# fraunhoferhhi/vvdec

Measured on AMD Instinct MI355X. Metric: decoded frames/sec (4K 10-bit RA) on MI355X, synthetic pre-parsed stream, bit-exact vs ref, higher is better.
Workload: dtype int16

## Files before the change

### vvdec_amd/csrc/vvr_api.cpp

```cpp
#include "vvr_host.h"
#include <algorithm>
#include <condition_variable>
#include <cstdio>
#include <cstring>
#include <deque>
#include <map>
#include <memory>
#include <mutex>
#include <thread>
#include <sched.h>
#include <pthread.h>

int vvr_upload_tables();

static std::vector<int> gpuNodeCpus( int device )
{
  std::vector<int> cpus;
  if( const char* e = getenv( "VVR_NO_PIN" ) ) if( atoi( e ) ) return cpus;
  char bus[64] = { 0 };
  if( hipDeviceGetPCIBusId( bus, sizeof( bus ), device ) != hipSuccess ) return cpus;
  for( char* q = bus; *q; q++ ) *q = (char) tolower( *q );
  char path[256]; snprintf( path, sizeof( path ), "/sys/bus/pci/devices/%s/numa_node", bus );
  int node = -1;
  if( FILE* f = fopen( path, "r" ) ) { if( fscanf( f, "%d", &node ) != 1 ) node = -1; fclose( f ); }
// ... 64 lines not shown
  int state = J_QUEUED;
  int rc = VVR_OK; std::string err;
  vvr_picture pic;
  vvr_prepared* q = nullptr;
  RingEntry* ring = nullptr;
  int lane = -1;
  hipEvent_t done = nullptr;
  hipEvent_t doneHost = nullptr;
  bool completed = false, waited = false;
  std::vector<PendingTiming> timings;
  int* errWord = nullptr;
  std::vector<int32_t> dmvr;
  std::vector<vvr_motion> col;
  bool handled = false;
#ifdef VVR_WATCHDOG
  double tSubmit = 0, tPrep = 0, tBuilt = 0, tRing = 0, tReady = 0, tCommit0 = 0, tCommit1 = 0; hipEvent_t tlA = nullptr, tlB = nullptr; int tlPoc = 0, tlType = 0; unsigned long long tlSeq = 0;
#endif
};

struct vvr_context {
  vvr_config cfg;
  int        device = 0;
  std::string err;
  std::vector<hipStream_t> streams;
  hipStream_t copyStream = nullptr;
  std::vector<DevPlanes>   slots;
  std::vector<std::pair<uint16_t, uint16_t>> slotDim;
  std::vector<DevPlanes>   scratchB;
  std::vector<DevPlanes>   scratchR;
  void*      planeMem = nullptr; bool planeMemOwned = false;
  void*      scratchMem = nullptr;
// ... 83 lines not shown

static hipEvent_t takeEvent( vvr_context* c )
{
  if( !c->eventPool.empty() ) { hipEvent_t e = c->eventPool.back(); c->eventPool.pop_back(); return e; }
  hipEvent_t e = nullptr;
  if( hipEventCreateWithFlags( &e, hipEventDisableTiming ) != hipSuccess ) return nullptr;
  return e;
}

static void completeLocked( vvr_context* c, Job& j )
{
  if( j.completed ) return;
#ifdef VVR_WATCHDOG
  if( j.tlA && j.tlB && c->tlBase )
  {
    float a = 0, b = 0; hipEventElapsedTime( &a, c->tlBase, j.tlA ); hipEventElapsedTime( &b, c->tlBase, j.tlB );
    fprintf( stderr, "[vvr timeline] device seq %3llu poc %4d type %d lane %d: %6.2f .. %6.2f  (base event recorded at host %6.2f)\n", j.tlSeq, j.tlPoc, j.tlType, j.lane, a, b, c->tlBaseHost - c->tl0 );
  }
  if( j.tlA ) { hipEventDestroy( j.tlA ); j.tlA = nullptr; } if( j.tlB ) { hipEventDestroy( j.tlB ); j.tlB = nullptr; }
#endif
  for( auto& t : j.timings )
  {
    float ms = 0; hipEventElapsedTime( &ms, t.a, t.b );
    c->stats[t.kernel].launches++; c->stats[t.kernel].ms += ms; c->stats[t.kernel].bytes += t.bytes;
    hipEventDestroy( t.a ); hipEventDestroy( t.b );
  }
  j.timings.clear();
  if( j.errWord && *j.errWord )
  {
    *j.errWord = 0;
    if( j.state == J_COMMITTED ) { j.state = J_FAILED; j.rc = VVR_ERR_DEVICE; j.err = "intra stage: a block waited for its neighbours beyond the bound (dependency that never completed)"; }
  }
  if( j.q && j.q->numDmvr && j.state == J_COMMITTED )
  {
    const int32_t* src = j.ring ? j.ring->dmvrHost : j.q->dmvrHost;
    j.dmvr.assign( src, src + 2 * (size_t) j.q->numDmvr );
  }
  if( j.q && j.q->colHost && j.state == J_COMMITTED ) j.col.assign( j.q->colHost, j.q->colHost + j.q->numCol );
  if( j.ring && j.ring->owner == &j ) { j.ring->owner = nullptr; j.ring->turn += c->ring.size(); }
  if( j.done ) { c->eventPool.push_back( j.done ); j.done = nullptr; }
  if( j.doneHost ) { c->eventPool.push_back( j.doneHost ); j.doneHost = nullptr; }
  j.q = nullptr;
  j.completed = true;
  WD_PROGRESS();
  c->cv.notify_all();
}

struct CommitPlan { int lane; std::vector<hipEvent_t> waits; RefSet refs; std::vector<int> waitInfo; std::vector<hipEvent_t> outExt ; };

static void pruneExternalEventsLocked( vvr_context* c, int slot )
{
  auto& v = c->slotExt[slot];
  v.erase( std::remove_if( v.begin(), v.end(), []( hipEvent_t ev ) { return hipEventQuery( ev ) == hipSuccess; } ), v.end() );
}

static void planCommitLocked( vvr_context* c, Job& job, CommitPlan& plan )
{
  const vvr_pic_header& h = job.q->hdr;
  int lane = -1;
  if( c->prioLane >= 0 && h.slice_type == 2 )
  {
    auto it = c->jobs.find( c->prioJob );
    bool idle = it == c->jobs.end() || it->second->completed;
// ... 4 lines not shown
  plan.lane = lane; plan.waits.clear(); plan.waitInfo.clear();
  job.lane = lane;
  auto waitFor = [&]( int id ) { auto it = c->jobs.find( id ); if( it != c->jobs.end() ) { Job& j = *it->second; if( !j.completed && j.state == J_COMMITTED && j.lane != lane ) { plan.waits.push_back( j.done ); plan.waitInfo.push_back( j.q ? ( j.id * 16 + j.q->hdr.slice_type * 4 ) : -1 ); plan.waitInfo.push_back( j.lane ); } } };
  for( int id : c->slotUsers[h.out_slot] ) waitFor( id );
  plan.outExt.clear();
  for( hipEvent_t ev : c->slotExt[h.out_slot] ) { plan.waits.push_back( ev ); plan.waitInfo.push_back( -2 ); plan.waitInfo.push_back( -1 ); plan.outExt.push_back( ev ); }
  memset( &plan.refs, 0, sizeof( plan.refs ) );
  if( h.slice_type != 2 )
    for( int l = 0; l < 2; l++ ) for( int i = 0; i < h.num_ref[l]; i++ )
    {
      const int slot = h.ref_slot[l][i];
      if( !c->slotUsers[slot].empty() ) waitFor( c->slotUsers[slot][0] );
      for( hipEvent_t ev : c->slotExt[slot] ) if( std::find( plan.waits.begin(), plan.waits.end(), ev ) == plan.waits.end() ) { plan.waits.push_back( ev ); plan.waitInfo.push_back( -2 ); plan.waitInfo.push_back( -1 ); }
      for( int k = 0; k < 3; k++ ) plan.refs.p[l * VVR_MAX_REFS + i][k] = c->slots[slot].p[k];
    }
  job.done = takeEvent( c ); job.doneHost = takeEvent( c );
}

static int enqueuePicture( vvr_context* c, Job& job, const CommitPlan& plan, std::string& err )
{
#undef HIPCHK
#define HIPCHK( ctx, call ) do { hipError_t e_ = ( call ); if( e_ != hipSuccess ) { err = std::string( #call ) + ": " + hipGetErrorString( e_ ); hipStreamSynchronize( ( ctx )->copyStream ); hipStreamSynchronize( ( ctx )->streams[plan.lane] ); return VVR_ERR_DEVICE; } } while( 0 )
  vvr_prepared* q = job.q;
  const vvr_pic_header& h = q->hdr;
  const int lane = plan.lane;
  hipStream_t s = c->streams[lane];
  if( !job.done || !job.doneHost ) { err = "hipEventCreate failed"; return VVR_ERR_DEVICE; }
#ifdef VVR_WATCHDOG
  const double wdA = wdNow();
#endif
  if( job.ring )
  {
    RingEntry& e = *job.ring;
    HIPCHK( c, hipMemcpyAsync( e.dev + e.stagedBegin, e.host + e.stagedBegin, e.stagedEnd - e.stagedBegin, hipMemcpyHostToDevice, c->copyStream ) );
    for( auto& d : e.direct ) HIPCHK( c, hipMemcpyAsync( e.dev + d.off, d.src, d.n, hipMemcpyHostToDevice, c->copyStream ) );
    HIPCHK( c, hipEventRecord( e.copied, c->copyStream ) );
    HIPCHK( c, hipStreamWaitEvent( s, e.copied, 0 ) );
  }
#ifdef VVR_WATCHDOG
  const double wdB = wdNow(); g_wdPart[0] += wdB - wdA; g_wdPartMax[0] = std::max( g_wdPartMax[0], wdB - wdA );
#endif
#ifdef VVR_WATCHDOG
  for( size_t wi = 0; wi < plan.waits.size(); wi++ )
  {
    const double w0 = wdNow(); HIPCHK( c, hipStreamWaitEvent( s, plan.waits[wi], 0 ) ); const double w = wdNow() - w0;
    if( w > 0.5 ) fprintf( stderr, "[vvr] slow wait: picture %d (type %d, lane %d) wait %zu of %zu on job %d (type %d, lane %d): %.2f ms\n", job.id, (int) h.slice_type, lane, wi, plan.waits.size(), plan.waitInfo[2 * wi] >> 4, ( plan.waitInfo[2 * wi] >> 2 ) & 3, plan.waitInfo[2 * wi + 1], w );
  }
#else
  for( hipEvent_t ev : plan.waits ) HIPCHK( c, hipStreamWaitEvent( s, ev, 0 ) );
#endif
#ifdef VVR_WATCHDOG
  const double wdC = wdNow(); g_wdPart[1] += wdC - wdB; g_wdPartMax[1] = std::max( g_wdPartMax[1], wdC - wdB );
  static const bool tlOn = getenv( "VVR_TIMELINE" ) != nullptr;
  if( tlOn && job.ring )
  {
    if( job.tSubmit - c->tl0 > 50 )
    {
      static hipStream_t tlStream = nullptr; if( !tlStream ) hipStreamCreate( &tlStream );
      c->tl0 = job.tSubmit; hipEventCreate( &c->tlBase ); hipEventRecord( c->tlBase, tlStream ); c->tlBaseHost = wdNow();
      fprintf( stderr, "[vvr timeline] ---- (host: ms since the first submit of the burst; device: ms since the base event)\n" );
    }
    hipEventCreate( &job.tlA ); hipEventCreate( &job.tlB ); job.tlPoc = h.poc; job.tlType = h.slice_type; job.tlSeq = job.seq;
    hipEventRecord( job.tlA, s );
  }
#endif
  job.errWord = c->errHost + ( (unsigned) job.id % VVR_ERR_WORDS ); *job.errWord = 0;
  const RefSet& refs = plan.refs;
  DevPlanes A = c->slots[h.out_slot], B = c->scratchB[lane], R = c->scratchR[lane];
  for( int k = 0; k < 3; k++ ) { const int w = k ? h.width >> 1 : h.width, hh = k ? h.height >> 1 : h.height; A.w[k] = B.w[k] = R.w[k] = w; A.h[k] = B.h[k] = R.h[k] = hh; }
  const int stopAfter = c->cfg.stop_after;
  const bool sao = ( h.tool_flags & ( VVR_TOOL_SAO_LUMA | VVR_TOOL_SAO_CHROMA ) ) != 0 && stopAfter != 1 && stopAfter != 2;
  const bool alf = ( h.tool_flags & VVR_TOOL_ALF ) != 0 && stopAfter == 0;
  const bool fused = ( sao || alf ) && sao_alf_fused( q->pic );
  const bool dbOn = !( h.tool_flags & VVR_TOOL_DEBLOCK_OFF ) && stopAfter != 1;
  const bool hop = fused && dbOn;
  const DevPlanes P = ( fused && !hop ) ? B : A;
  auto timedOn = [&]( int k, hipStream_t st, double algoBytes, auto&& fn )
  {
#ifdef VVR_WATCHDOG
    static const int skipMask = getenv( "VVR_SKIP_KERNELS" ) ? atoi( getenv( "VVR_SKIP_KERNELS" ) ) : 0;
    if( skipMask & ( 1 << k ) ) return;
    const double w0 = wdNow();
#endif
    if( c->statsOn ) { PendingTiming t; hipEventCreate( &t.a ); hipEventCreate( &t.b ); t.kernel = k; t.bytes = algoBytes; hipEventRecord( t.a, st ); fn(); hipEventRecord( t.b, st ); job.timings.push_back( t ); }
    else fn();
#ifdef VVR_WATCHDOG
    const double w = wdNow() - w0; g_wdCall[k][0] += w; g_wdCall[k][1] = std::max( g_wdCall[k][1], w ); g_wdCall[k][2] += 1;
#endif
  };
  auto timed = [&]( int k, auto&& fn ) { timedOn( k, s, q->bytes[k], fn ); };
  {
    PrepWork w;
    if( q->numMcCus ) { w.mcCus = q->mcCus; w.numMcCus = q->numMcCus; w.plain = q->mcDev; w.bdof = q->bdofItems; w.dmvr = q->dmvrItems; }
    if( q->lfpOnDevice && dbOn ) { w.lfMaps = true; w.numCu = q->numCu; w.numTu = q->numTu; w.cell = q->lfCell; w.cellC = q->lfCellC; w.mv = q->lfMv; w.ref = q->lfRef; w.sb = q->lfSb; w.numSb = q->numLfSb; }
    if( q->intraLeaf && q->numIntra ) { w.items = q->intraItems; w.numItems = q->numIntra; w.resi = q->resiItems; w.numResi = q->numResi; w.maps = c->leafMaps[lane]; w.mapInts = c->leafMapInts; w.mapW4 = c->leafW4; w.mapH4 = c->leafH4; }
    launch_prep( s, q->pic, w );
  }
  if( q->lfpOnDevice && dbOn ) timed( K_LF_INIT, [&]{ launch_lf_init( s, q->pic, q->numCu, q->numTu, q->lfCell, q->lfCellC, q->lfMv, q->lfRef, q->lfSb, q->numLfSb, q->lfpDev[0], q->lfpDev[1] ); } );
  if( q->numMc + q->numMcDev ) timedOn( K_MC, s, q->bytes[K_MC] - q->bytesBdof, [&]{ launch_mc( s, q->pic, refs, P, q->mcItems, q->numMc, q->mcDev, q->numMcDev, 0 ); } );
  if( q->numBdofItems ) timedOn( K_MC, s, q->bytesBdof, [&]{ launch_mc( s, q->pic, refs, P, nullptr, 0, q->bdofItems, q->numBdofItems, 1 ); } );
  if( q->numDmvrItems )
  {
    int32_t* out = job.ring ? job.ring->dmvrHost : q->dmvrHost;
    memset( out, 0, sizeof( int32_t ) * 2 * (size_t) q->numDmvr );
    timed( K_MC_DMVR, [&]{ launch_mc_dmvr( s, q->pic, refs, P, q->dmvrItems, q->numDmvrItems, out ); } );
  }
  if( q->numAffItems ) timed( K_MC_AFFINE, [&]{ launch_mc_affine( s, q->pic, refs, P, q->affItems, q->numAffItems ); } );
  if( q->numRprItems ) launch_mc_rpr( s, q->pic, refs, P, q->rprItems, q->numRprItems );
  const bool lmcsOn = ( h.tool_flags & VVR_TOOL_LMCS ) != 0;
  for( int k = 0; k < 3; k++ ) if( q->numTb[k] ) timedOn( K_ITRANS, s, q->bytesTb[k], [&]{ launch_itrans( s, q->pic, P, R, q->tbItems[k], q->numTb[k], 16 << k ); } );
  {
    const size_t need = q->intraLeaf ? 0 : intra_sync_ints( q->numActive, q->numIntra );
    if( need > c->syncCap[lane] )
// ... 313 lines not shown
    for( size_t i = 0; i < c->ring.size(); i++ ) fprintf( stderr, "  ring %zu owner %d\n", i, c->ring[i].owner ? c->ring[i].owner->id : -1 );
    for( size_t i = 0; i < c->streams.size(); i++ ) fprintf( stderr, "  stream %zu query %d\n", i, (int) hipStreamQuery( c->streams[i] ) );
    fprintf( stderr, "  copyStream query %d\n", (int) hipStreamQuery( c->copyStream ) );
    fflush( stderr );
    abort();
  }
}
#endif

struct WorkerHelpers : HostHelpers
{
  vvr_context* c; PrepScratch*& spare;
  bool announced = false;
  WorkerHelpers( vvr_context* c_, PrepScratch*& spare_ ) : c( c_ ), spare( spare_ ) {}
  int width() const override { return c->cfg.host_threads; }
  void notInParts() override { if( announced ) { std::lock_guard<std::mutex> lk( c->mu ); c->partsComing--; announced = false; c->cv.notify_all(); } }
  void run( int n, PrepScratch& own, const std::function<void( int, PrepScratch& )>& fn ) override
  {
    struct State { std::mutex mu; std::condition_variable cv; int remaining; } st; st.remaining = n - 1;
    {
      std::lock_guard<std::mutex> lk( c->mu );
      const bool first = announced;
      for( int part = first ? n - 1 : 1; first ? part >= 1 : part < n; part += first ? -1 : 1 )
      {
        auto task = [&st, &fn, part]( PrepScratch& R ) { fn( part, R ); std::lock_guard<std::mutex> l2( st.mu ); st.remaining--; st.cv.notify_all(); };
        if( first ) c->subtasks.push_front( task ); else c->subtasks.push_back( task );
      }
      if( announced ) { c->partsComing--; announced = false; }
      c->cv.notify_all();
    }
    fn( 0, own );
    for( ;; )
    {
      std::function<void( PrepScratch& )> task;
      { std::lock_guard<std::mutex> lk( c->mu ); if( !c->subtasks.empty() ) { task = std::move( c->subtasks.front() ); c->subtasks.pop_front(); } }
      if( !task ) break;
      if( !spare ) { spare = vvr_scratch_create(); vvr_scratch_intra_leaf( spare, c->intraLeaf, c->leafByLevel ); vvr_scratch_warm( spare, c->cfg ); }
      task( *spare );
    }
    std::unique_lock<std::mutex> lk( st.mu );
    st.cv.wait( lk, [&]{ return st.remaining == 0; } );
  }
};
// ... 662 lines not shown
```

### vvdec_amd/csrc/vvr_host.h

```cpp
#pragma once
#include "vvr_device.h"
#include <mutex>
#include <string>
#include <vector>

static inline size_t alignUp( size_t v, size_t a ) { return ( v + a - 1 ) / a * a; }

enum { K_MC, K_MC_DMVR, K_MC_AFFINE, K_LMCS, K_ITRANS, K_INTRA, K_RESI_ADD, K_DEBLOCK_V, K_DEBLOCK_H, K_SAO, K_ALF, K_COPY, K_OUTPUT, K_LF_INIT, K_INTRA_LEAF,
       K_DEBLOCK4, K_ALF_PLANES ,
       K_OUTPUT_FRAME , K_NUM };

struct vvr_prepared {
  vvr_pic_header hdr;
  PicDev   pic;
  McItem*  mcItems = nullptr; int numMc = 0;
  McItem*  mcDev = nullptr; int numMcDev = 0;
  McCuRef* mcCus = nullptr; int numMcCus = 0;
  McItem*  bdofItems = nullptr; int numBdofItems = 0;
  McItem*  dmvrItems = nullptr; int numDmvrItems = 0;
  McItem*  affItems = nullptr; int numAffItems = 0;
  McItem*  rprItems = nullptr; int numRprItems = 0;
  uint32_t numDmvr = 0;
  TbItem*  tbItems[3] = { nullptr, nullptr, nullptr }; int numTb[3] = { 0, 0, 0 };
  IntraItem* intraItems = nullptr; IntraUnit* units = nullptr; int numActive = 0, numIntra = 0;
// ... 32 lines not shown
int          vvr_host_band_pictures();
void         vvr_scratch_intra_leaf( PrepScratch*, bool on, bool byLevel = false );
void         vvr_scratch_parts_for_all( PrepScratch*, bool on );
void         vvr_scratch_destroy( PrepScratch* );
void         vvr_scratch_warm( PrepScratch*, const vvr_config& cfg );

int    vvr_host_validate( const vvr_config& cfg, const vvr_picture* p, std::string& err );
int    vvr_host_validate_header( const vvr_config& cfg, const vvr_picture* p, std::string& err );
int    vvr_host_validate_records( const vvr_config& cfg, const vvr_picture* p, std::string& err );
#include <functional>
struct HostHelpers
{
  virtual ~HostHelpers() {}
  virtual int  width() const = 0;
  virtual void run( int n, PrepScratch& own, const std::function<void( int, PrepScratch& )>& fn ) = 0;
  virtual void notInParts() {}
};
int    vvr_host_build( const vvr_picture* p, PrepScratch& S, size_t* totalBytes, std::string& err, PinnedRanges* pinned = nullptr, HostHelpers* helpers = nullptr, bool validateRecords = false );
void   vvr_host_pack( const PrepScratch& S, char* host );
size_t vvr_host_staged_bytes( const PrepScratch& S );
size_t vvr_host_num_col( const vvr_picture* p );
void   vvr_host_gather_col( const vvr_picture* p, vvr_motion* dst );
void   vvr_host_upload_plan( const PrepScratch& S, std::vector<DirectCopy>& direct, size_t* stagedBegin, size_t* stagedEnd );
void   vvr_host_bind( const PrepScratch& S, vvr_prepared& q, char* devBase );
```

### vvdec_amd/csrc/vvr_prepare.cpp

```cpp
#include "vvr_host.h"
#include "vvr_lf_init.h"
#include <algorithm>
#include <atomic>
#include <chrono>
#include <cstdio>
#include <cstring>
#include <mutex>
#include <condition_variable>

static inline int ilog2i( int v ) { int l = 0; while( ( 1 << l ) < v ) l++; return l; }

struct BBox { int y0 = 255, y1 = 0, c0 = 255, c1 = 0; };
struct ItemH { uint32_t ctu; BBox bb; uint32_t p0, pn; };
struct DepList
{
  enum { INLINE = 8 };
  uint32_t n = 0, cap = INLINE; uint32_t in[INLINE]; uint32_t* heap = nullptr;
  DepList() {}
  DepList( const DepList& o ) { *this = o; }
  DepList( DepList&& o ) noexcept { n = o.n; cap = o.cap; heap = o.heap; memcpy( in, o.in, sizeof( in ) ); o.heap = nullptr; o.n = 0; o.cap = INLINE; }
  DepList& operator=( const DepList& o ) { if( this != &o ) { n = 0; for( uint32_t v : o ) push_back( v ); } return *this; }
  DepList& operator=( DepList&& o ) noexcept { if( this != &o ) { delete[] heap; n = o.n; cap = o.cap; heap = o.heap; memcpy( in, o.in, sizeof( in ) ); o.heap = nullptr; o.n = 0; o.cap = INLINE; } return *this; }
  ~DepList() { delete[] heap; }
  uint32_t* data() { return heap ? heap : in; } const uint32_t* data() const { return heap ? heap : in; }
  uint32_t* begin() { return data(); } uint32_t* end() { return data() + n; } const uint32_t* begin() const { return data(); } const uint32_t* end() const { return data() + n; }
  size_t size() const { return n; } bool empty() const { return n == 0; }
  uint32_t& operator[]( size_t i ) { return data()[i]; } const uint32_t& operator[]( size_t i ) const { return data()[i]; }
  void push_back( uint32_t v ) { if( n == cap ) { uint32_t* h = new uint32_t[2 * cap]; memcpy( h, data(), sizeof( uint32_t ) * n ); delete[] heap; heap = h; cap *= 2; } data()[n++] = v; }
  void resize( size_t k ) { n = (uint32_t) std::min<size_t>( k, n ); }
  void assign( const uint32_t* a, const uint32_t* b ) { n = 0; for( ; a != b; a++ ) push_back( *a ); }
  void clear() { n = 0; }
};
struct UnitH { uint32_t comp, ctu, i0, i1, iA = 0; bool hasCs = false; BBox bb; DepList deps; bool waited = false; int rank = 0; };

struct Part { const void* src; size_t n, off; bool direct; };

struct PrepScratch
{
  const vvr_picture* p = nullptr;
  vvr_pic_header h;
  int ncomp = 0, w4 = 0, h4 = 0, ctu = 0, ctusX = 0, ctusY = 0, numCtu = 0, vpduLog2 = 0, vpdusX = 0, vpdusY = 0;
  bool wpOn = false, cscale = false, lmcs = false;
  std::vector<McItem> mcRpr;
  std::vector<McItem> mc, mcBdof, mcDmvr, mcAff;
  std::vector<McCuRef> mcCus;
  uint32_t devTiles[3] = { 0, 0, 0 };
  std::vector<uint16_t> ctuSubpicV;
  std::vector<vvr_motion> affMv;
  bool lfpOnDevice = false;
  std::vector<LfSbCell> lfSb;
// ... 7 lines not shown
  std::vector<uint32_t> ctuStartV;
  double bytes[K_NUM] = { 0 };
  double bytesBdof = 0, bytesIntraLuma = 0, bytesTb[3] = { 0, 0, 0 };
  std::vector<int32_t> order;
  std::vector<uint8_t> fastCtu;
  std::vector<uint32_t> itemAtE[3];
  uint16_t fastCell[3][32 * 32]; uint32_t fastFirst[3] = { 0, 0, 0 };
  uint32_t epoch = 0;
  size_t cellIdx( int cx, int cy ) const { const int l = h.log2_ctu - 2, m = ( 1 << l ) - 1; return ( ( (size_t) ( cy >> l ) * ctusX + ( cx >> l ) ) << ( 2 * l ) ) | (size_t) ( ( cy & m ) << l ) | (size_t) ( cx & m ); }
  int32_t itemAtGet( int k, size_t cell ) const { const uint32_t v = itemAtE[k][cell]; return ( v >> 22 ) == epoch ? (int32_t) ( v & 0x3fffffu ) : -1; }
  std::vector<UnitH> units, unitsTmp;
  std::vector<uint32_t> csVpduV;
  std::vector<std::pair<uint32_t, uint32_t>> csProdRange;
  std::vector<uint32_t> csProdPool;
  std::vector<IntraUnit> unitsDev;
  int intraWorkgroups = 0, intraWorkgroupsChroma = 0, numLumaUnits = 0;
  std::vector<IntraItem> resiAdd;
  size_t intraChunk = (size_t) 1 << 30;
  std::vector<uint32_t> parent, newIdx, firstOf, perm, inv, unitCount, unitOfItem[3];
  std::vector<uint64_t> sortKey;
  std::vector<int32_t> unitOfRoot, target;
  std::vector<std::vector<uint32_t>> members, groups;
  std::vector<Part> parts;
  size_t total = 0, numDirect = 0;
  int iLfSb, iLfTu, iLfTuC, iLfMotion;
  int iCu, iTu, iCoef, iAffMv, iL0, iL1, iSao, iAlf, iAlfP, iSlices, iLmcs, iSl, iCtuSlice, iCtuTile, iSubpics, iCtuSubpic, iWp, iCsVpdu, iMc, iMcB, iMcD, iMcA, iTb[3], iIntra, iResi, iUnits, iMcCus, iMcDev[3], iRpr, iMcR;
  size_t stagedEndOff = 0;

  void begin( const vvr_picture* pic )
  {
// ... 6 lines not shown
    {
      uint32_t any = 0;
      for( uint32_t i = 0; i < p->num_slices; i++ ) any |= p->slices[i].tool_flags & VVR_SLICE_TOOL_MASK;
      h.tool_flags = ( h.tool_flags & ~(uint32_t) VVR_SLICE_TOOL_MASK ) | any;
    }
    wpOn = ( h.tool_flags & VVR_TOOL_WP ) && h.slice_type != 2;
    w4 = ( h.width + 3 ) >> 2; h4 = ( h.height + 3 ) >> 2; ctu = 1 << h.log2_ctu;
    ctusX = ( h.width + ctu - 1 ) / ctu; ctusY = ( h.height + ctu - 1 ) / ctu; numCtu = ctusX * ctusY;
    lmcs = ( h.tool_flags & VVR_TOOL_LMCS ) != 0;
    cscale = lmcs && ( h.tool_flags & VVR_TOOL_LMCS_CSCALE ) && ncomp == 3;
    vpduLog2 = std::min<int>( 6, h.log2_ctu ); vpdusX = ( h.width + ( 1 << vpduLog2 ) - 1 ) >> vpduLog2; vpdusY = ( h.height + ( 1 << vpduLog2 ) - 1 ) >> vpduLog2;
    mc.clear(); mcBdof.clear(); mcDmvr.clear(); mcAff.clear(); mcRpr.clear(); affMv.clear(); numDmvr = 0;
    lfSb.clear(); lfpOnDevice = ( h.tool_flags & VVR_TOOL_LFP_ON_DEVICE ) && !( h.tool_flags & VVR_TOOL_DEBLOCK_OFF );
    mcCus.clear(); devTiles[0] = devTiles[1] = devTiles[2] = 0;
    for( int k = 0; k < 3; k++ ) { tb[k].clear(); intra[k].clear(); itemH[k].clear(); prodPool[k].clear(); }
    resiAdd.clear(); intraAll.clear(); units.clear(); unitsDev.clear(); csVpduV.clear(); intraFine = false;
    ctuStartV.assign( 3 * (size_t) ( numCtu + 1 ), 0 );
    for( double& b : bytes ) b = 0;
    bytesBdof = bytesIntraLuma = 0; bytesTb[0] = bytesTb[1] = bytesTb[2] = 0;
  }

  size_t orderIdx( int chn, int lx, int ly ) const { const int m = ( 1 << ( h.log2_ctu - 2 ) ) - 1; return ( ( (size_t) chn << ( h.log2_ctu - 2 ) | (size_t) ( ( ly >> 2 ) & m ) ) << ( h.log2_ctu - 2 ) ) | (size_t) ( ( lx >> 2 ) & m ); }
  int unitAvail( int chn, int x, int y, int32_t cur ) const
  {
    const int cs = chn ? 1 : 0, lx = x << cs, ly = y << cs;
    if( x < 0 || y < 0 || lx >= h.width || ly >= h.height ) return 0;
    const uint32_t c = (uint32_t) ( ( ly >> h.log2_ctu ) * ctusX + ( lx >> h.log2_ctu ) );
    if( c != curCtuIdx ) return c < curCtuIdx && sameSliceAndTile( c, curCtuIdx );
    return order[orderIdx( chn, lx, ly )] < cur;
  }

// ... 43 lines not shown
  inline void levLook( int k, int cx0, int cy0, int cx1, int cy1, uint32_t& d ) const
  {
    cx0 = std::max( cx0, 0 ); cy0 = std::max( cy0, 0 ); cx1 = std::min( cx1, w4 - 1 ); cy1 = std::min( cy1, h4 - 1 );
    const uint16_t* m = &levMap[(size_t) k * w4 * h4];
    for( int y = cy0; y <= cy1; y++ ) for( int x = cx0; x <= cx1; x++ ) d = std::max<uint32_t>( d, m[(size_t) y * w4 + x] );
  }
  inline void levOwn( int k, int cx0, int cy0, int cx1, int cy1, uint16_t v )
  {
    cx1 = std::min( cx1, w4 - 1 ); cy1 = std::min( cy1, h4 - 1 );
    uint16_t* m = &levMap[(size_t) k * w4 * h4];
    for( int y = cy0; y <= cy1; y++ ) std::fill( m + (size_t) y * w4 + cx0, m + (size_t) y * w4 + cx1 + 1, v );
  }
  int emitLeafItems( std::string& err );
  int buildWorkLists( std::string& err, uint32_t cu0 = 0, uint32_t cu1 = 0xffffffffu );
  int buildInParts( const vvr_config& cfg, HostHelpers& helpers, bool validate, std::string& err );
  int formUnits();
  int groupUnits();
  int emitUnitTable( std::string& err );
  void layout( PinnedRanges* pinned );
  void foldLongDepLists();
  void rankUnits();
};

PrepScratch* vvr_scratch_create() { return new PrepScratch(); }
void vvr_scratch_parts_for_all( PrepScratch* S, bool on ) { S->partsForAll = on; }
void vvr_scratch_intra_leaf( PrepScratch* S, bool on, bool byLevel ) { S->leafOn = on; S->leafSortOn = byLevel; }
static bool tusAreTheSplitAt32( const vvr_picture* p, const vvr_cu& cu )
{
  const int tw = cu.w < 32 ? cu.w : 32, th = cu.h < 32 ? cu.h : 32, nx = cu.w / tw, ny = cu.h / th;
  if( (int) cu.num_tu != nx * ny || cu.num_tu < 2 ) return false;
// ... 1144 lines not shown
  {
    UnitH& U = merged[newIndexOfGroup[m]];
    for( uint32_t u : groups[m] ) for( uint32_t d : units[u].deps )
    {
      const uint32_t nd = newIndexOfGroup[target[d]];
      if( nd != newIndexOfGroup[m] && std::find( U.deps.begin(), U.deps.end(), nd ) == U.deps.end() ) U.deps.push_back( nd );
    }
  }
  for( int k = 0; k < ncomp; k++ ) intra[k].swap( intraTmp[k] );
  units.swap( merged );
  foldLongDepLists();
  rankUnits();
  return VVR_OK;
}

int PrepScratch::emitUnitTable( std::string& err )
{
  auto bandsLog2 = [&]( const IntraItem& src, int k )
  {
    const int samples = 1 << ( src.lw + src.lh );
    const bool split = samples > IT_SPLIT_SAMPLES && src.mode <= 66 && ( k || ( !( src.flags & IT_F_MIP ) && ( src.flags & IT_F_ISP ) != IT_F_ISP ) );
    int lp = 0;
    if( split ) while( lp < IT_MAX_LPARTS && ( samples >> lp ) > IT_SPLIT_SAMPLES ) lp++;
    return lp;
  };
  {
    uint32_t at = (uint32_t) intraAll.size();
    for( int k = 0; k < 3; k++ )
    {
      const size_t n = intra[k].size();
      itemMap[k].resize( n + 1 );
      uint32_t* im = itemMap[k].data(); const IntraItem* src = intra[k].data();
      for( size_t bi = 0; bi < n; bi++ ) { im[bi] = at; at += 1u << bandsLog2( src[bi], k ); }
      im[n] = at;
    }
    intraAll.resize( at );
  }
  for( int k = 0; k < 3; k++ )
  {
    const size_t n = intra[k].size();
    const uint32_t* im = itemMap[k].data(); const IntraItem* srcs = intra[k].data(); IntraItem* out = intraAll.data();
    for( size_t bi = 0; bi < n; bi++ )
    {
      const IntraItem& src = srcs[bi];
      const uint32_t indepBlocks = std::min<uint32_t>( src.comp >> 2, (uint32_t) bi );
      const uint32_t indepItems = im[bi] - im[bi - indepBlocks];
      const int lp = ilog2i( (int) ( im[bi + 1] - im[bi] ) );
      for( int part = 0; part < ( 1 << lp ); part++ )
      {
        IntraItem it = src;
        it.nTL = (uint8_t) ( ( src.nTL & 1 ) | ( part << 1 ) | ( lp << 4 ) );
        it.comp = (uint8_t) ( k | ( std::min<uint32_t>( 63, indepItems + part ) << 2 ) );
        out[im[bi] + part] = it;
// ... 174 lines not shown
  for( int k = 0; k < 3; k++ ) iMcDev[k] = add( nullptr, sizeof( McItem ) * devTiles[k] );
  iLfTu = iLfTuC = iLfMotion = -1;
  if( lfpOnDevice )
  {
    const size_t cells = (size_t) w4 * h4;
    iL0 = add( nullptr, sizeof( vvr_lfp ) * cells ); iL1 = add( nullptr, sizeof( vvr_lfp ) * cells );
    iLfTu = add( nullptr, sizeof( LfCell ) * cells ); iLfTuC = ncomp == 3 ? add( nullptr, sizeof( LfCell ) * cells ) : -1;
    iLfMotion = add( nullptr, ( sizeof( LfMv ) + sizeof( uint32_t ) ) * cells );
    bytes[K_LF_INIT] = (double) cells * ( 2 * sizeof( LfCell ) + ( h.slice_type != 2 ? sizeof( vvr_motion ) : 0 ) + 2 * sizeof( vvr_lfp ) ) + (double) sizeof( vvr_cu ) * p->num_cu + (double) sizeof( vvr_tu ) * p->num_tu + (double) lfSb.size() * sizeof( LfSbCell );
  }
}

int PrepScratch::buildInParts( const vvr_config& cfg, HostHelpers& helpers, bool validate, std::string& err )
{
  (void) cfg;
  const int n = std::min( helpers.width(), ctusY );
  struct Shared { std::mutex mu; std::condition_variable cv; int turn = 0; int rc = VVR_OK; std::string err; uint64_t area[2] = { 0, 0 }; } sh;
  const vvr_picture* pic = p;
  PrepScratch* owner = this;
  const bool analysed = !allIntraCus && !leaf;
  if( !allIntraCus ) g_bandPictures++;
  if( analysed ) for( int k = 0; k < ncomp; k++ ) edgeRow[k].assign( (size_t) w4, -1 );
  helpers.run( n, *this, [&]( int part, PrepScratch& R )
  {
    const int row0 = (int) ( (int64_t) owner->ctusY * part / n ), row1 = (int) ( (int64_t) owner->ctusY * ( part + 1 ) / n );
    const uint32_t cu0 = pic->ctu_first_cu[(size_t) row0 * owner->ctusX], cu1 = pic->ctu_first_cu[(size_t) row1 * owner->ctusX];
    int rc = VVR_OK; std::string e; uint64_t area[2] = { 0, 0 };
    if( cu0 > cu1 || cu1 > pic->num_cu ) { rc = VVR_ERR_PARAMETER; e = "ctu_first_cu is not ascending"; }
    if( rc == VVR_OK && validate ) rc = validate_records_range( pic, cu0, cu1, area, e );
    if( rc == VVR_OK )
// ... 74 lines not shown
      }
      if( analysed && part + 1 < n )
      {
        const int cy = ( std::min( row1 << O.h.log2_ctu, (int) O.h.height ) - 1 ) >> 2;
        for( int k = 0; k < O.ncomp; k++ ) for( int cx = 0; cx < O.w4; cx++ ) { const int32_t d = R.itemAtGet( k, R.cellIdx( cx, cy ) ); O.edgeRow[k][cx] = d < 0 ? -1 : d + (int32_t) off[k]; }
      }
    }
    sh.turn = part + 1;
    sh.cv.notify_all();
  } );
  if( sh.rc != VVR_OK ) { err = sh.err; return sh.rc; }
  if( validate ) return validate_cover( p, sh.area, err );
  return VVR_OK;
}

int vvr_host_build( const vvr_picture* p, PrepScratch& S, size_t* totalBytes, std::string& err, PinnedRanges* pinned, HostHelpers* helpers, bool validateRecords )
{
  S.begin( p );
  int rc;
  const bool anyInParts = S.partsForAll && !p->rpr;
  if( helpers && helpers->width() > 1 && !( p->hdr.tool_flags & VVR_TOOL_IBC ) && p->ctu_first_cu && p->num_cu >= 512 && S.ctusY >= 2 && ( p->hdr.slice_type == 2 || anyInParts ) )
  {
    if( ( rc = S.beginMaps() ) != VVR_OK ) return rc;
    if( S.allIntraCus || anyInParts )
    {
      if( ( rc = S.buildInParts( vvr_config(), *helpers, validateRecords, err ) ) != VVR_OK ) return rc;
      if( S.leaf ) { if( ( rc = S.emitLeafItems( err ) ) != VVR_OK ) return rc; }
      else if( ( rc = S.formUnits() ) != VVR_OK || ( rc = S.groupUnits() ) != VVR_OK || ( rc = S.emitUnitTable( err ) ) != VVR_OK ) return rc;
      S.layout( pinned );
      *totalBytes = S.total;
      return VVR_OK;
    }
  }
  if( helpers ) helpers->notInParts();
  if( validateRecords && ( rc = vvr_host_validate_records( vvr_config(), p, err ) ) != VVR_OK ) return rc;
#ifdef VVR_DEV_ENV
  if( getenv( "VVR_PHASES" ) )
  {
    auto now = []{ return std::chrono::duration<double, std::milli>( std::chrono::steady_clock::now().time_since_epoch() ).count(); };
    double t[7]; t[0] = now();
    rc = S.beginMaps(); S.beginLevels(); t[1] = now();
    if( rc == VVR_OK ) rc = S.buildWorkLists( err ); t[2] = now();
    if( rc == VVR_OK && !S.leaf ) rc = S.formUnits(); t[3] = now();
    if( rc == VVR_OK && !S.leaf ) rc = S.groupUnits(); t[4] = now();
// ... 93 lines not shown
```

Measured before the change: 2588.

## Parallelise intra-picture host build in bands and defer cross-lane waits past prep

Adds a dedicated banded build for all-intra pictures. Each helper thread builds its band's work lists and unit headers. After a join, a second parallel phase expands intra items and copies TBs while one task forms and groups units. On the device side, a picture's prep and LF-init kernels are now enqueued before the reference and output-slot event waits, with a new front wait only on jobs sharing the same prepared buffer, so front-end kernels can overlap earlier pictures. This adds complexity and a risk of ordering bugs if the prep kernels touch state that the deferred waits protected.

```diff
diff --git a/vvdec_amd/csrc/vvr_api.cpp b/vvdec_amd/csrc/vvr_api.cpp
--- a/vvdec_amd/csrc/vvr_api.cpp
+++ b/vvdec_amd/csrc/vvr_api.cpp
@@ -102,7 +102,7 @@
   std::vector<vvr_motion> col;
   bool handled = false;
 #ifdef VVR_WATCHDOG
-  double tSubmit = 0, tPrep = 0, tBuilt = 0, tRing = 0, tReady = 0, tCommit0 = 0, tCommit1 = 0; hipEvent_t tlA = nullptr, tlB = nullptr; int tlPoc = 0, tlType = 0; unsigned long long tlSeq = 0;
+  double tSubmit = 0, tPrep = 0, tBuilt = 0, tRing = 0, tReady = 0, tCommit0 = 0, tCommit1 = 0; hipEvent_t tlF = nullptr , tlA = nullptr , tlB = nullptr; int tlPoc = 0, tlType = 0; unsigned long long tlSeq = 0;
 #endif
 };
 
@@ -216,10 +216,10 @@
 #ifdef VVR_WATCHDOG
   if( j.tlA && j.tlB && c->tlBase )
   {
-    float a = 0, b = 0; hipEventElapsedTime( &a, c->tlBase, j.tlA ); hipEventElapsedTime( &b, c->tlBase, j.tlB );
-    fprintf( stderr, "[vvr timeline] device seq %3llu poc %4d type %d lane %d: %6.2f .. %6.2f  (base event recorded at host %6.2f)\n", j.tlSeq, j.tlPoc, j.tlType, j.lane, a, b, c->tlBaseHost - c->tl0 );
-  }
-  if( j.tlA ) { hipEventDestroy( j.tlA ); j.tlA = nullptr; } if( j.tlB ) { hipEventDestroy( j.tlB ); j.tlB = nullptr; }
+    float f = 0, a = 0, b = 0; if( j.tlF ) hipEventElapsedTime( &f, c->tlBase, j.tlF ); hipEventElapsedTime( &a, c->tlBase, j.tlA ); hipEventElapsedTime( &b, c->tlBase, j.tlB );
+    fprintf( stderr, "[vvr timeline] device seq %3llu poc %4d type %d lane %d: front %6.2f  %6.2f .. %6.2f  (base event recorded at host %6.2f)\n", j.tlSeq, j.tlPoc, j.tlType, j.lane, f, a, b, c->tlBaseHost - c->tl0 );
+  }
+  if( j.tlF ) { hipEventDestroy( j.tlF ); j.tlF = nullptr; } if( j.tlA ) { hipEventDestroy( j.tlA ); j.tlA = nullptr; } if( j.tlB ) { hipEventDestroy( j.tlB ); j.tlB = nullptr; }
 #endif
   for( auto& t : j.timings )
   {
@@ -248,7 +248,8 @@
   c->cv.notify_all();
 }
 
-struct CommitPlan { int lane; std::vector<hipEvent_t> waits; RefSet refs; std::vector<int> waitInfo; std::vector<hipEvent_t> outExt ; };
+struct CommitPlan { int lane; std::vector<hipEvent_t> waits; RefSet refs; std::vector<int> waitInfo; std::vector<hipEvent_t> outExt ;
+                    std::vector<hipEvent_t> frontWaits ; };
 
 static void pruneExternalEventsLocked( vvr_context* c, int slot )
 {
@@ -283,6 +284,9 @@
       for( hipEvent_t ev : c->slotExt[slot] ) if( std::find( plan.waits.begin(), plan.waits.end(), ev ) == plan.waits.end() ) { plan.waits.push_back( ev ); plan.waitInfo.push_back( -2 ); plan.waitInfo.push_back( -1 ); }
       for( int k = 0; k < 3; k++ ) plan.refs.p[l * VVR_MAX_REFS + i][k] = c->slots[slot].p[k];
     }
+  plan.frontWaits.clear();
+  if( !job.ring )
+    for( auto& kv : c->jobs ) { const Job& j = *kv.second; if( &j != &job && j.q == job.q && !j.completed && j.state == J_COMMITTED && j.lane != lane && j.done ) plan.frontWaits.push_back( j.done ); }
   job.done = takeEvent( c ); job.doneHost = takeEvent( c );
 }
 
@@ -309,17 +313,23 @@
 #ifdef VVR_WATCHDOG
   const double wdB = wdNow(); g_wdPart[0] += wdB - wdA; g_wdPartMax[0] = std::max( g_wdPartMax[0], wdB - wdA );
 #endif
-#ifdef VVR_WATCHDOG
-  for( size_t wi = 0; wi < plan.waits.size(); wi++ )
-  {
-    const double w0 = wdNow(); HIPCHK( c, hipStreamWaitEvent( s, plan.waits[wi], 0 ) ); const double w = wdNow() - w0;
-    if( w > 0.5 ) fprintf( stderr, "[vvr] slow wait: picture %d (type %d, lane %d) wait %zu of %zu on job %d (type %d, lane %d): %.2f ms\n", job.id, (int) h.slice_type, lane, wi, plan.waits.size(), plan.waitInfo[2 * wi] >> 4, ( plan.waitInfo[2 * wi] >> 2 ) & 3, plan.waitInfo[2 * wi + 1], w );
-  }
-#else
-  for( hipEvent_t ev : plan.waits ) HIPCHK( c, hipStreamWaitEvent( s, ev, 0 ) );
-#endif
-#ifdef VVR_WATCHDOG
-  const double wdC = wdNow(); g_wdPart[1] += wdC - wdB; g_wdPartMax[1] = std::max( g_wdPartMax[1], wdC - wdB );
+  const int stopAfter = c->cfg.stop_after;
+  const bool dbOn = !( h.tool_flags & VVR_TOOL_DEBLOCK_OFF ) && stopAfter != 1;
+  auto timedOn = [&]( int k, hipStream_t st, double algoBytes, auto&& fn )
+  {
+#ifdef VVR_WATCHDOG
+    static const int skipMask = getenv( "VVR_SKIP_KERNELS" ) ? atoi( getenv( "VVR_SKIP_KERNELS" ) ) : 0;
+    if( skipMask & ( 1 << k ) ) return;
+    const double w0 = wdNow();
+#endif
+    if( c->statsOn ) { PendingTiming t; hipEventCreate( &t.a ); hipEventCreate( &t.b ); t.kernel = k; t.bytes = algoBytes; hipEventRecord( t.a, st ); fn(); hipEventRecord( t.b, st ); job.timings.push_back( t ); }
+    else fn();
+#ifdef VVR_WATCHDOG
+    const double w = wdNow() - w0; g_wdCall[k][0] += w; g_wdCall[k][1] = std::max( g_wdCall[k][1], w ); g_wdCall[k][2] += 1;
+#endif
+  };
+  auto timed = [&]( int k, auto&& fn ) { timedOn( k, s, q->bytes[k], fn ); };
+#ifdef VVR_WATCHDOG
   static const bool tlOn = getenv( "VVR_TIMELINE" ) != nullptr;
   if( tlOn && job.ring )
   {
@@ -329,35 +339,11 @@
       c->tl0 = job.tSubmit; hipEventCreate( &c->tlBase ); hipEventRecord( c->tlBase, tlStream ); c->tlBaseHost = wdNow();
       fprintf( stderr, "[vvr timeline] ---- (host: ms since the first submit of the burst; device: ms since the base event)\n" );
     }
-    hipEventCreate( &job.tlA ); hipEventCreate( &job.tlB ); job.tlPoc = h.poc; job.tlType = h.slice_type; job.tlSeq = job.seq;
-    hipEventRecord( job.tlA, s );
-  }
-#endif
-  job.errWord = c->errHost + ( (unsigned) job.id % VVR_ERR_WORDS ); *job.errWord = 0;
-  const RefSet& refs = plan.refs;
-  DevPlanes A = c->slots[h.out_slot], B = c->scratchB[lane], R = c->scratchR[lane];
-  for( int k = 0; k < 3; k++ ) { const int w = k ? h.width >> 1 : h.width, hh = k ? h.height >> 1 : h.height; A.w[k] = B.w[k] = R.w[k] = w; A.h[k] = B.h[k] = R.h[k] = hh; }
-  const int stopAfter = c->cfg.stop_after;
-  const bool sao = ( h.tool_flags & ( VVR_TOOL_SAO_LUMA | VVR_TOOL_SAO_CHROMA ) ) != 0 && stopAfter != 1 && stopAfter != 2;
-  const bool alf = ( h.tool_flags & VVR_TOOL_ALF ) != 0 && stopAfter == 0;
-  const bool fused = ( sao || alf ) && sao_alf_fused( q->pic );
-  const bool dbOn = !( h.tool_flags & VVR_TOOL_DEBLOCK_OFF ) && stopAfter != 1;
-  const bool hop = fused && dbOn;
-  const DevPlanes P = ( fused && !hop ) ? B : A;
-  auto timedOn = [&]( int k, hipStream_t st, double algoBytes, auto&& fn )
-  {
-#ifdef VVR_WATCHDOG
-    static const int skipMask = getenv( "VVR_SKIP_KERNELS" ) ? atoi( getenv( "VVR_SKIP_KERNELS" ) ) : 0;
-    if( skipMask & ( 1 << k ) ) return;
-    const double w0 = wdNow();
-#endif
-    if( c->statsOn ) { PendingTiming t; hipEventCreate( &t.a ); hipEventCreate( &t.b ); t.kernel = k; t.bytes = algoBytes; hipEventRecord( t.a, st ); fn(); hipEventRecord( t.b, st ); job.timings.push_back( t ); }
-    else fn();
-#ifdef VVR_WATCHDOG
-    const double w = wdNow() - w0; g_wdCall[k][0] += w; g_wdCall[k][1] = std::max( g_wdCall[k][1], w ); g_wdCall[k][2] += 1;
-#endif
-  };
-  auto timed = [&]( int k, auto&& fn ) { timedOn( k, s, q->bytes[k], fn ); };
+    hipEventCreate( &job.tlF ); hipEventCreate( &job.tlA ); hipEventCreate( &job.tlB ); job.tlPoc = h.poc; job.tlType = h.slice_type; job.tlSeq = job.seq;
+    hipEventRecord( job.tlF, s );
+  }
+#endif
+  for( hipEvent_t ev : plan.frontWaits ) HIPCHK( c, hipStreamWaitEvent( s, ev, 0 ) );
   {
     PrepWork w;
     if( q->numMcCus ) { w.mcCus = q->mcCus; w.numMcCus = q->numMcCus; w.plain = q->mcDev; w.bdof = q->bdofItems; w.dmvr = q->dmvrItems; }
@@ -366,6 +352,28 @@
     launch_prep( s, q->pic, w );
   }
   if( q->lfpOnDevice && dbOn ) timed( K_LF_INIT, [&]{ launch_lf_init( s, q->pic, q->numCu, q->numTu, q->lfCell, q->lfCellC, q->lfMv, q->lfRef, q->lfSb, q->numLfSb, q->lfpDev[0], q->lfpDev[1] ); } );
+#ifdef VVR_WATCHDOG
+  for( size_t wi = 0; wi < plan.waits.size(); wi++ )
+  {
+    const double w0 = wdNow(); HIPCHK( c, hipStreamWaitEvent( s, plan.waits[wi], 0 ) ); const double w = wdNow() - w0;
+    if( w > 0.5 ) fprintf( stderr, "[vvr] slow wait: picture %d (type %d, lane %d) wait %zu of %zu on job %d (type %d, lane %d): %.2f ms\n", job.id, (int) h.slice_type, lane, wi, plan.waits.size(), plan.waitInfo[2 * wi] >> 4, ( plan.waitInfo[2 * wi] >> 2 ) & 3, plan.waitInfo[2 * wi + 1], w );
+  }
+#else
+  for( hipEvent_t ev : plan.waits ) HIPCHK( c, hipStreamWaitEvent( s, ev, 0 ) );
+#endif
+#ifdef VVR_WATCHDOG
+  const double wdC = wdNow(); g_wdPart[1] += wdC - wdB; g_wdPartMax[1] = std::max( g_wdPartMax[1], wdC - wdB );
+  if( job.tlA ) hipEventRecord( job.tlA, s );
+#endif
+  job.errWord = c->errHost + ( (unsigned) job.id % VVR_ERR_WORDS ); *job.errWord = 0;
+  const RefSet& refs = plan.refs;
+  DevPlanes A = c->slots[h.out_slot], B = c->scratchB[lane], R = c->scratchR[lane];
+  for( int k = 0; k < 3; k++ ) { const int w = k ? h.width >> 1 : h.width, hh = k ? h.height >> 1 : h.height; A.w[k] = B.w[k] = R.w[k] = w; A.h[k] = B.h[k] = R.h[k] = hh; }
+  const bool sao = ( h.tool_flags & ( VVR_TOOL_SAO_LUMA | VVR_TOOL_SAO_CHROMA ) ) != 0 && stopAfter != 1 && stopAfter != 2;
+  const bool alf = ( h.tool_flags & VVR_TOOL_ALF ) != 0 && stopAfter == 0;
+  const bool fused = ( sao || alf ) && sao_alf_fused( q->pic );
+  const bool hop = fused && dbOn;
+  const DevPlanes P = ( fused && !hop ) ? B : A;
   if( q->numMc + q->numMcDev ) timedOn( K_MC, s, q->bytes[K_MC] - q->bytesBdof, [&]{ launch_mc( s, q->pic, refs, P, q->mcItems, q->numMc, q->mcDev, q->numMcDev, 0 ); } );
   if( q->numBdofItems ) timedOn( K_MC, s, q->bytesBdof, [&]{ launch_mc( s, q->pic, refs, P, nullptr, 0, q->bdofItems, q->numBdofItems, 1 ); } );
   if( q->numDmvrItems )
@@ -709,6 +717,8 @@
   bool announced = false;
   WorkerHelpers( vvr_context* c_, PrepScratch*& spare_ ) : c( c_ ), spare( spare_ ) {}
   int width() const override { return c->cfg.host_threads; }
+  bool again = false;
+  void partsFollow() override { again = true; }
   void notInParts() override { if( announced ) { std::lock_guard<std::mutex> lk( c->mu ); c->partsComing--; announced = false; c->cv.notify_all(); } }
   void run( int n, PrepScratch& own, const std::function<void( int, PrepScratch& )>& fn ) override
   {
@@ -721,7 +731,8 @@
         auto task = [&st, &fn, part]( PrepScratch& R ) { fn( part, R ); std::lock_guard<std::mutex> l2( st.mu ); st.remaining--; st.cv.notify_all(); };
         if( first ) c->subtasks.push_front( task ); else c->subtasks.push_back( task );
       }
-      if( announced ) { c->partsComing--; announced = false; }
+      if( again ) { if( !announced ) { c->partsComing++; announced = true; } again = false; }
+      else if( announced ) { c->partsComing--; announced = false; }
       c->cv.notify_all();
     }
     fn( 0, own );
diff --git a/vvdec_amd/csrc/vvr_host.h b/vvdec_amd/csrc/vvr_host.h
--- a/vvdec_amd/csrc/vvr_host.h
+++ b/vvdec_amd/csrc/vvr_host.h
@@ -70,6 +70,7 @@
   virtual ~HostHelpers() {}
   virtual int  width() const = 0;
   virtual void run( int n, PrepScratch& own, const std::function<void( int, PrepScratch& )>& fn ) = 0;
+  virtual void partsFollow() {}
   virtual void notInParts() {}
 };
 int    vvr_host_build( const vvr_picture* p, PrepScratch& S, size_t* totalBytes, std::string& err, PinnedRanges* pinned = nullptr, HostHelpers* helpers = nullptr, bool validateRecords = false );
diff --git a/vvdec_amd/csrc/vvr_prepare.cpp b/vvdec_amd/csrc/vvr_prepare.cpp
--- a/vvdec_amd/csrc/vvr_prepare.cpp
+++ b/vvdec_amd/csrc/vvr_prepare.cpp
@@ -34,6 +34,18 @@
 struct UnitH { uint32_t comp, ctu, i0, i1, iA = 0; bool hasCs = false; BBox bb; DepList deps; bool waited = false; int rank = 0; };
 
 struct Part { const void* src; size_t n, off; bool direct; };
+
+struct IntraPartOut
+{
+  int rc = VVR_OK; std::string err; uint64_t area[2] = { 0, 0 };
+  std::vector<IntraItem> intra[3];
+  std::vector<TbItem> tb[3];
+  std::vector<UnitH> units[3];
+  std::vector<uint32_t> im[3];
+  double bytes[K_NUM], bytesBdof = 0, bytesIntraLuma = 0, bytesTb[3];
+  uint32_t blockOff[3], itemOff[3], tbOff[3];
+  double tDone = 0;
+};
 
 struct PrepScratch
 {
@@ -71,6 +83,9 @@
   std::vector<std::pair<uint32_t, uint32_t>> csProdRange;
   std::vector<uint32_t> csProdPool;
   std::vector<IntraUnit> unitsDev;
+  std::vector<IntraPartOut> partOut;
+  bool fromParts = false;
+  double phaseT[4] = { 0, 0, 0, 0 };
   int intraWorkgroups = 0, intraWorkgroupsChroma = 0, numLumaUnits = 0;
   std::vector<IntraItem> resiAdd;
   size_t intraChunk = (size_t) 1 << 30;
@@ -107,7 +122,7 @@
     lfSb.clear(); lfpOnDevice = ( h.tool_flags & VVR_TOOL_LFP_ON_DEVICE ) && !( h.tool_flags & VVR_TOOL_DEBLOCK_OFF );
     mcCus.clear(); devTiles[0] = devTiles[1] = devTiles[2] = 0;
     for( int k = 0; k < 3; k++ ) { tb[k].clear(); intra[k].clear(); itemH[k].clear(); prodPool[k].clear(); }
-    resiAdd.clear(); intraAll.clear(); units.clear(); unitsDev.clear(); csVpduV.clear(); intraFine = false;
+    resiAdd.clear(); intraAll.clear(); units.clear(); unitsDev.clear(); csVpduV.clear(); intraFine = false; fromParts = false;
     ctuStartV.assign( 3 * (size_t) ( numCtu + 1 ), 0 );
     for( double& b : bytes ) b = 0;
     bytesBdof = bytesIntraLuma = 0; bytesTb[0] = bytesTb[1] = bytesTb[2] = 0;
@@ -181,6 +196,7 @@
   int emitLeafItems( std::string& err );
   int buildWorkLists( std::string& err, uint32_t cu0 = 0, uint32_t cu1 = 0xffffffffu );
   int buildInParts( const vvr_config& cfg, HostHelpers& helpers, bool validate, std::string& err );
+  int buildIntraInParts( HostHelpers& helpers, bool validate, std::string& err );
   int formUnits();
   int groupUnits();
   int emitUnitTable( std::string& err );
@@ -1355,16 +1371,18 @@
   return VVR_OK;
 }
 
+static inline int bandsLog2( const IntraItem& src, int k )
+{
+  const int samples = 1 << ( src.lw + src.lh );
+  const bool split = samples > IT_SPLIT_SAMPLES && src.mode <= 66 && ( k || ( !( src.flags & IT_F_MIP ) && ( src.flags & IT_F_ISP ) != IT_F_ISP ) );
+  int lp = 0;
+  if( split ) while( lp < IT_MAX_LPARTS && ( samples >> lp ) > IT_SPLIT_SAMPLES ) lp++;
+  return lp;
+}
+
 int PrepScratch::emitUnitTable( std::string& err )
 {
-  auto bandsLog2 = [&]( const IntraItem& src, int k )
-  {
-    const int samples = 1 << ( src.lw + src.lh );
-    const bool split = samples > IT_SPLIT_SAMPLES && src.mode <= 66 && ( k || ( !( src.flags & IT_F_MIP ) && ( src.flags & IT_F_ISP ) != IT_F_ISP ) );
-    int lp = 0;
-    if( split ) while( lp < IT_MAX_LPARTS && ( samples >> lp ) > IT_SPLIT_SAMPLES ) lp++;
-    return lp;
-  };
+  if( !fromParts )
   {
     uint32_t at = (uint32_t) intraAll.size();
     for( int k = 0; k < 3; k++ )
@@ -1377,7 +1395,7 @@
     }
     intraAll.resize( at );
   }
-  for( int k = 0; k < 3; k++ )
+  for( int k = 0; k < 3 && !fromParts; k++ )
   {
     const size_t n = intra[k].size();
     const uint32_t* im = itemMap[k].data(); const IntraItem* srcs = intra[k].data(); IntraItem* out = intraAll.data();
@@ -1582,6 +1600,7 @@
 int PrepScratch::buildInParts( const vvr_config& cfg, HostHelpers& helpers, bool validate, std::string& err )
 {
   (void) cfg;
+  if( allIntraCus && intraChunk == (size_t) 1 << 30 ) return buildIntraInParts( helpers, validate, err );
   const int n = std::min( helpers.width(), ctusY );
   struct Shared { std::mutex mu; std::condition_variable cv; int turn = 0; int rc = VVR_OK; std::string err; uint64_t area[2] = { 0, 0 }; } sh;
   const vvr_picture* pic = p;
@@ -1686,6 +1705,171 @@
   return VVR_OK;
 }
 
+static inline double phaseNow() { return std::chrono::duration<double, std::milli>( std::chrono::steady_clock::now().time_since_epoch() ).count(); }
+
+int PrepScratch::buildIntraInParts( HostHelpers& helpers, bool validate, std::string& err )
+{
+  const int n = std::min( helpers.width(), ctusY );
+  const vvr_picture* pic = p;
+  PrepScratch* owner = this;
+  if( partOut.size() < (size_t) n ) partOut.resize( (size_t) n );
+#if defined( VVR_WATCHDOG ) || defined( VVR_DEV_ENV )
+  phaseT[0] = phaseNow();
+#endif
+  helpers.partsFollow();
+  helpers.run( n, *this, [&]( int part, PrepScratch& R )
+  {
+    PrepScratch& O = *owner;
+    IntraPartOut& PO = O.partOut[(size_t) part];
+    const int row0 = (int) ( (int64_t) O.ctusY * part / n ), row1 = (int) ( (int64_t) O.ctusY * ( part + 1 ) / n );
+    const uint32_t cu0 = pic->ctu_first_cu[(size_t) row0 * O.ctusX], cu1 = pic->ctu_first_cu[(size_t) row1 * O.ctusX];
+    int rc = VVR_OK; std::string e;
+    PO.area[0] = PO.area[1] = 0;
+    if( cu0 > cu1 || cu1 > pic->num_cu ) { rc = VVR_ERR_PARAMETER; e = "ctu_first_cu is not ascending"; }
+    if( rc == VVR_OK && validate ) rc = validate_records_range( pic, cu0, cu1, PO.area, e );
+    if( rc == VVR_OK )
+    {
+      if( &R != owner ) { R.begin( pic ); rc = R.beginMaps( owner ); }
+      R.partCtu0 = (uint32_t) row0 * O.ctusX; R.partCtu1 = (uint32_t) row1 * O.ctusX;
+      R.partTopY = 0; R.partBad = false; R.pending.clear();
+      if( rc == VVR_OK ) rc = R.buildWorkLists( e, cu0, cu1 );
+      R.partCtu0 = 0; R.partCtu1 = 0xffffffffu;
+      if( rc == VVR_OK && !( R.mc.empty() && R.mcBdof.empty() && R.mcDmvr.empty() && R.mcAff.empty() && R.mcRpr.empty() && R.mcCus.empty() && R.lfSb.empty() && R.resiAdd.empty() ) )
+        { rc = VVR_ERR_UNSPECIFIED; e = "internal: inter-stage work in a picture of intra CUs"; }
+    }
+    if( rc == VVR_OK )
+    {
+      for( int k = 0; k < 3; k++ )
+      {
+        std::vector<UnitH>& U = PO.units[k]; U.clear();
+        std::vector<uint32_t>& im = PO.im[k];
+        const size_t nb = k < O.ncomp ? R.intra[k].size() : 0;
+        im.resize( nb + 1 );
+        const ItemH* IH = R.itemH[k].data(); const IntraItem* IT = R.intra[k].data();
+        uint32_t at = 0;
+        for( size_t i = 0; i < nb; )
+        {
+          UnitH u; u.comp = (uint32_t) k; u.ctu = IH[i].ctu; u.i0 = (uint32_t) i;
+          for( ; i < nb && IH[i].ctu == u.ctu; i++ )
+          {
+            const BBox& b = IH[i].bb;
+            u.bb.y0 = std::min( u.bb.y0, b.y0 ); u.bb.y1 = std::max( u.bb.y1, b.y1 ); u.bb.c0 = std::min( u.bb.c0, b.c0 ); u.bb.c1 = std::max( u.bb.c1, b.c1 );
+            if( k && ( IT[i].flags & IT_F_CSCALE ) ) u.hasCs = true;
+            im[i] = at; at += 1u << bandsLog2( IT[i], k );
+          }
+          u.i1 = (uint32_t) i; u.iA = u.i0;
+          U.push_back( std::move( u ) );
+        }
+        im[nb] = at;
+        if( k < O.ncomp ) PO.intra[k].swap( R.intra[k] ); else PO.intra[k].clear();
+        PO.tb[k].swap( R.tb[k] );
+      }
+      memcpy( PO.bytes, R.bytes, sizeof( PO.bytes ) ); PO.bytesBdof = R.bytesBdof; PO.bytesIntraLuma = R.bytesIntraLuma; for( int k = 0; k < 3; k++ ) PO.bytesTb[k] = R.bytesTb[k];
+      if( &R != owner )
+      {
+        for( uint32_t c = (uint32_t) row0 * O.ctusX; c < (uint32_t) row1 * O.ctusX; c++ ) O.fastCtu[c] = R.fastCtu[c];
+        if( O.cscale )
+        {
+          const int nv = 1 << ( O.h.log2_ctu - O.vpduLog2 );
+          const size_t v0 = (size_t) row0 * nv * O.vpdusX, v1 = std::min( (size_t) row1 * nv, (size_t) O.vpdusY ) * O.vpdusX;
+          if( v1 > v0 ) memcpy( &O.csVpduV[v0], &R.csVpduV[v0], sizeof( uint32_t ) * ( v1 - v0 ) );
+        }
+      }
+    }
+    PO.rc = rc; PO.err.swap( e );
+#if defined( VVR_WATCHDOG ) || defined( VVR_DEV_ENV )
+    PO.tDone = phaseNow();
+#endif
+  } );
+  uint64_t area[2] = { 0, 0 };
+  for( int part = 0; part < n; part++ )
+  {
+    IntraPartOut& PO = partOut[(size_t) part];
+    if( PO.rc != VVR_OK ) { helpers.notInParts(); err = PO.err; return PO.rc; }
+    area[0] += PO.area[0]; area[1] += PO.area[1];
+  }
+#if defined( VVR_WATCHDOG ) || defined( VVR_DEV_ENV )
+  phaseT[1] = phaseT[0]; for( int part = 0; part < n; part++ ) phaseT[1] = std::max( phaseT[1], partOut[(size_t) part].tDone );
+#endif
+  {
+    uint32_t items = 0;
+    for( int k = 0; k < 3; k++ )
+    {
+      uint32_t blocks = 0, tbs = 0;
+      for( int part = 0; part < n; part++ )
+      {
+        IntraPartOut& PO = partOut[(size_t) part];
+        PO.blockOff[k] = blocks; PO.itemOff[k] = items; PO.tbOff[k] = tbs;
+        blocks += (uint32_t) PO.intra[k].size(); items += PO.im[k].back(); tbs += (uint32_t) PO.tb[k].size();
+      }
+      intra[k].clear();
+      itemMap[k].resize( (size_t) blocks + 1 );
+      tb[k].resize( tbs );
+      for( int part = 0; part < n; part++ )
+      {
+        const IntraPartOut& PO = partOut[(size_t) part];
+        for( const UnitH& pu : PO.units[k] )
+        {
+          itemMap[k][PO.blockOff[k] + pu.i0] = PO.itemOff[k] + PO.im[k][pu.i0]; itemMap[k][PO.blockOff[k] + pu.i1] = PO.itemOff[k] + PO.im[k][pu.i1];
+          units.push_back( pu );
+          UnitH& u = units.back(); u.i0 += PO.blockOff[k]; u.i1 += PO.blockOff[k]; u.iA = u.i0;
+        }
+      }
+    }
+    intraAll.resize( items );
+    for( int part = 0; part < n; part++ )
+    {
+      const IntraPartOut& PO = partOut[(size_t) part];
+      for( int k = 0; k < K_NUM; k++ ) bytes[k] = part ? bytes[k] + PO.bytes[k] : PO.bytes[k];
+      bytesIntraLuma = part ? bytesIntraLuma + PO.bytesIntraLuma : PO.bytesIntraLuma; bytesBdof = part ? bytesBdof + PO.bytesBdof : PO.bytesBdof;
+      for( int k = 0; k < 3; k++ ) bytesTb[k] = part ? bytesTb[k] + PO.bytesTb[k] : PO.bytesTb[k];
+    }
+    fromParts = true;
+  }
+#if defined( VVR_WATCHDOG ) || defined( VVR_DEV_ENV )
+  phaseT[2] = phaseNow();
+#endif
+  int rcUnits = VVR_OK; std::string errUnits;
+  helpers.run( n + 1, *this, [&]( int task, PrepScratch& )
+  {
+    PrepScratch& O = *owner;
+    if( task == 0 )
+    {
+      if( ( rcUnits = O.formUnits() ) == VVR_OK && ( rcUnits = O.groupUnits() ) == VVR_OK ) rcUnits = O.emitUnitTable( errUnits );
+      return;
+    }
+    IntraPartOut& PO = O.partOut[(size_t) task - 1];
+    for( int k = 0; k < 3; k++ )
+    {
+      const size_t nb = PO.intra[k].size();
+      const uint32_t* im = PO.im[k].data(); const IntraItem* srcs = PO.intra[k].data(); IntraItem* out = O.intraAll.data() + PO.itemOff[k];
+      for( size_t bi = 0; bi < nb; bi++ )
+      {
+        const IntraItem& src = srcs[bi];
+        uint32_t indepBlocks = src.comp >> 2;
+        if( indepBlocks > bi ) { if( PO.blockOff[k] ) { PO.rc = VVR_ERR_UNSPECIFIED; PO.err = "internal: a block's independent predecessors reach into the band above"; } indepBlocks = (uint32_t) bi; }
+        const uint32_t indepItems = im[bi] - im[bi - indepBlocks];
+        const int lp = ilog2i( (int) ( im[bi + 1] - im[bi] ) );
+        for( int part = 0; part < ( 1 << lp ); part++ )
+        {
+          IntraItem it = src;
+          it.nTL = (uint8_t) ( ( src.nTL & 1 ) | ( part << 1 ) | ( lp << 4 ) );
+          it.comp = (uint8_t) ( k | ( std::min<uint32_t>( 63, indepItems + part ) << 2 ) );
+          out[im[bi] + part] = it;
+        }
+      }
+      if( !PO.tb[k].empty() ) memcpy( O.tb[k].data() + PO.tbOff[k], PO.tb[k].data(), sizeof( TbItem ) * PO.tb[k].size() );
+    }
+  } );
+#if defined( VVR_WATCHDOG ) || defined( VVR_DEV_ENV )
+  phaseT[3] = phaseNow();
+#endif
+  for( int part = 0; part < n; part++ ) if( partOut[(size_t) part].rc != VVR_OK ) { err = partOut[(size_t) part].err; return partOut[(size_t) part].rc; }
+  if( rcUnits != VVR_OK ) { err = errUnits; return rcUnits; }
+  if( validate ) return validate_cover( p, area, err );
+  return VVR_OK;
+}
+
 int vvr_host_build( const vvr_picture* p, PrepScratch& S, size_t* totalBytes, std::string& err, PinnedRanges* pinned, HostHelpers* helpers, bool validateRecords )
 {
   S.begin( p );
@@ -1697,9 +1881,18 @@
     if( S.allIntraCus || anyInParts )
     {
       if( ( rc = S.buildInParts( vvr_config(), *helpers, validateRecords, err ) ) != VVR_OK ) return rc;
-      if( S.leaf ) { if( ( rc = S.emitLeafItems( err ) ) != VVR_OK ) return rc; }
+      if( S.fromParts ) {}
+      else if( S.leaf ) { if( ( rc = S.emitLeafItems( err ) ) != VVR_OK ) return rc; }
       else if( ( rc = S.formUnits() ) != VVR_OK || ( rc = S.groupUnits() ) != VVR_OK || ( rc = S.emitUnitTable( err ) ) != VVR_OK ) return rc;
       S.layout( pinned );
+#if defined( VVR_WATCHDOG ) || defined( VVR_DEV_ENV )
+      if( S.fromParts && ( getenv( "VVR_PHASES" ) || getenv( "VVR_TIMELINE" ) ) )
+      {
+        const double t = phaseNow();
+        fprintf( stderr, "[vvr] I picture in bands (ms): phase 1 %.3f, join %.3f, phase 2 and units %.3f, layout %.3f; last band through phase 1 -> built %.3f; stage %.3f\n",
+                 S.phaseT[1] - S.phaseT[0], S.phaseT[2] - S.phaseT[1], S.phaseT[3] - S.phaseT[2], t - S.phaseT[3], t - S.phaseT[1], t - S.phaseT[0] );
+      }
+#endif
       *totalBytes = S.total;
       return VVR_OK;
     }
```

New measurement: 2663 (median of 6 runs). 2.9% higher.
